# zju-pi/diff-sampler

Measured on NVIDIA H100. Metric: images/sec at fixed NFE, higher is better.
Workload: dtype fp16 operands, fp32 accumulate (split-precision: fp16 hi x hi + two e4m3 correction MMAs per product); 1 GPU; EDM cifar10 U-Net, heun num_steps=10 (NFE=18), batch 512/GPU; net=cifar10, solver=heun, nfe=18, batch_per_gpu=512, global_batch=512, weights=random init (reference constructors, seed 0), init_zero layers de-zeroed, parallelism=dp1, l2=per-forward activation working set (GBs) >> 50 MB L2

## Files before the change

### diff-sampler_b200/_cstructs.py

```python
import ctypes as C

P = C.c_uint64
I32 = C.c_int32
I64 = C.c_int64
F32 = C.c_float
F64 = C.c_double

DS_OP_GEMM, DS_OP_GN_STATS, DS_OP_GN_APPLY, DS_OP_SOFTMAX, DS_OP_POSEMB, DS_OP_LINEAR = 1, 2, 3, 4, 5, 6
DS_OP_PREP_INPUT, DS_OP_CHANMEAN, DS_OP_MEMSET, DS_OP_LAYERNORM, DS_OP_GEGLU, DS_OP_GN_FINALIZE, DS_OP_ATTN, DS_OP_EMBED = 7, 8, 9, 10, 11, 12, 13, 14
DS_OP_OPT_PREP, DS_OP_OPT_SOFTMAX, DS_OP_OPT_REDUCE, DS_OP_OPT_KNN = 15, 16, 17, 18
DS_OP_IMG_INPUT, DS_OP_IM2COL, DS_OP_POOL = 19, 20, 21
DS_OP_CLIP_INPUT, DS_OP_CLIP_HEAD = 22, 23
DS_OP_PRDC_KTH, DS_OP_PRDC_COUNT = 24, 25
DS_PRDC_KMAX, DS_PRDC_LIST = 63, 1024
DS_CLIP_GATHER, DS_CLIP_L2NORM, DS_CLIP_SCORE = 0, 1, 2
DS_POOL_MAX, DS_POOL_AVG, DS_POOL_MEAN = 0, 1, 2
DS_IO_X, DS_IO_D, DS_IO_SIGMA, DS_IO_LABELS, DS_IO_BOTTLENECK, DS_IO_CTX, DS_IO_COUNT = 0, 1, 2, 3, 4, 5, 6
DS_M_X0, DS_M_EPS, DS_M_DIV, DS_M_NONE = 0, 1, 2, 3
DS_F8_SH_A16, DS_F8_SH_LO8, DS_F8_SH_HI8 = 6, 13, 2
DS_OPT_CAP, DS_OPT_P_SHIFT, DS_OPT_BAND_NATS, DS_OPT_TAU, DS_OPT_EPS = 1024, 15, 40, 0.01, 2.0 ** -17
DS_OPT_PLAIN, DS_OPT_RESCORED, DS_OPT_UNREFINED = 0, 1, 2
DS_KNN_MAX, DS_KNN_CAND = 64, 256

SPACE_ABS, SPACE_ARENA, SPACE_WEIGHTS, SPACE_IO = 0, 1, 2, 3


def ref(space, offset):
    return (space << 60) | int(offset)


class GemmDesc(C.Structure):
    _fields_ = [
        ('a_ptr', P), ('a_dims', I64 * 4), ('a_strides', I64 * 3), ('a_box', I32 * 4), ('a_plane_n', I32),
        ('a2_ptr', P), ('a2_c', I64), ('a2_plane_n', I32), ('nkb_aux', I32),
        ('b_ptr', P), ('b_dims', I64 * 3), ('b_strides', I64 * 2), ('b_plane_batch', I32),
        ('BN', I32), ('m_tiles', I32), ('n_tiles', I32), ('num_z', I32), ('nh', I32),
# ... 104 lines not shown


class ClipInputDesc(C.Structure):
    _fields_ = [('src', P), ('tab', P), ('out', P), ('sn', I64), ('sc', I64), ('sy', I64), ('sx', I64), ('B', I32), ('H', I32), ('W', I32),
                ('S', I32), ('ky', I32), ('kx', I32), ('mean', F32 * 3), ('std', F32 * 3)]


class ClipHeadDesc(C.Structure):
    _fields_ = [('src', P), ('src2', P), ('ids', P), ('out', P), ('src_stride', I64), ('out_stride', I64), ('B', I32), ('C', I32), ('T', I32),
                ('row', I32), ('mode', I32), ('scale', F32)]


class PrdcKthDesc(C.Structure):
    _fields_ = [('part', P), ('q', P), ('t', P), ('qn2', P), ('tn2', P), ('rad', P), ('rad2', P), ('nres', P), ('ldp', I64),
                ('B', I32), ('N', I32), ('D', I32), ('nslice', I32), ('k', I32), ('pad0', I32), ('sq', F64), ('st', F64)]


class PrdcCountDesc(C.Structure):
    _fields_ = [('part', P), ('q', P), ('t', P), ('qn2', P), ('tn2', P), ('tau', P), ('tau2', P), ('rho', P), ('rho2', P), ('cnt_t', P),
                ('cnt_own', P), ('realism', P), ('nres', P), ('ldp', I64), ('B', I32), ('N', I32), ('D', I32), ('nslice', I32),
                ('sq', F64), ('st', F64), ('med', F64)]


class MemsetDesc(C.Structure):
    _fields_ = [('ptr', P), ('bytes', I64)]


class _OpUnion(C.Union):
    _fields_ = [('gemm', GemmDesc), ('gn_stats', GnStatsDesc), ('gn_apply', GnApplyDesc), ('softmax', SoftmaxDesc),
                ('posemb', PosembDesc), ('linear', LinearDesc), ('prep_input', PrepInputDesc), ('chanmean', ChanmeanDesc),
                ('memset', MemsetDesc), ('layernorm', LayernormDesc), ('geglu', GegluDesc), ('gn_finalize', GnFinalizeDesc), ('attn', AttnDesc),
                ('embed', EmbedDesc), ('opt_prep', OptPrepDesc), ('opt_softmax', OptSoftmaxDesc), ('opt_reduce', OptReduceDesc),
                ('opt_knn', OptKnnDesc), ('img_input', ImgInputDesc), ('im2col', Im2colDesc), ('pool', PoolDesc),
                ('clip_input', ClipInputDesc), ('clip_head', ClipHeadDesc), ('prdc_kth', PrdcKthDesc), ('prdc_count', PrdcCountDesc)]


class PlanOp(C.Structure):
    _fields_ = [('type', I32), ('tag', I32), ('u', _OpUnion)]


SIZEOF_CHECKS = {
    0: PlanOp, DS_OP_GEMM: GemmDesc, DS_OP_GN_STATS: GnStatsDesc, DS_OP_GN_APPLY: GnApplyDesc, DS_OP_SOFTMAX: SoftmaxDesc,
    DS_OP_POSEMB: PosembDesc, DS_OP_LINEAR: LinearDesc, DS_OP_PREP_INPUT: PrepInputDesc, DS_OP_CHANMEAN: ChanmeanDesc,
    DS_OP_MEMSET: MemsetDesc, DS_OP_LAYERNORM: LayernormDesc, DS_OP_GEGLU: GegluDesc, DS_OP_GN_FINALIZE: GnFinalizeDesc, DS_OP_ATTN: AttnDesc,
    DS_OP_EMBED: EmbedDesc, DS_OP_OPT_PREP: OptPrepDesc, DS_OP_OPT_SOFTMAX: OptSoftmaxDesc, DS_OP_OPT_REDUCE: OptReduceDesc,
    DS_OP_OPT_KNN: OptKnnDesc, DS_OP_IMG_INPUT: ImgInputDesc, DS_OP_IM2COL: Im2colDesc, DS_OP_POOL: PoolDesc,
    DS_OP_CLIP_INPUT: ClipInputDesc, DS_OP_CLIP_HEAD: ClipHeadDesc, DS_OP_PRDC_KTH: PrdcKthDesc, DS_OP_PRDC_COUNT: PrdcCountDesc,
}

UNION_FIELD = {
    DS_OP_GEMM: 'gemm', DS_OP_GN_STATS: 'gn_stats', DS_OP_GN_APPLY: 'gn_apply', DS_OP_SOFTMAX: 'softmax', DS_OP_POSEMB: 'posemb',
    DS_OP_LINEAR: 'linear', DS_OP_PREP_INPUT: 'prep_input', DS_OP_CHANMEAN: 'chanmean', DS_OP_MEMSET: 'memset',
    DS_OP_LAYERNORM: 'layernorm', DS_OP_GEGLU: 'geglu', DS_OP_GN_FINALIZE: 'gn_finalize', DS_OP_ATTN: 'attn', DS_OP_EMBED: 'embed',
}
OPT_UNION_FIELD = {DS_OP_OPT_PREP: 'opt_prep', DS_OP_OPT_SOFTMAX: 'opt_softmax', DS_OP_OPT_REDUCE: 'opt_reduce', DS_OP_OPT_KNN: 'opt_knn'}
INCEPTION_UNION_FIELD = {DS_OP_IMG_INPUT: 'img_input', DS_OP_IM2COL: 'im2col', DS_OP_POOL: 'pool'}
OPENCLIP_UNION_FIELD = {DS_OP_CLIP_INPUT: 'clip_input', DS_OP_CLIP_HEAD: 'clip_head'}
PRDC_UNION_FIELD = {DS_OP_PRDC_KTH: 'prdc_kth', DS_OP_PRDC_COUNT: 'prdc_count'}
ALL_UNION_FIELD = {**UNION_FIELD, **OPT_UNION_FIELD, **INCEPTION_UNION_FIELD, **OPENCLIP_UNION_FIELD, **PRDC_UNION_FIELD}
OP_TYPE_OF = {GemmDesc: DS_OP_GEMM, GnStatsDesc: DS_OP_GN_STATS, GnApplyDesc: DS_OP_GN_APPLY, SoftmaxDesc: DS_OP_SOFTMAX,
              PosembDesc: DS_OP_POSEMB, LinearDesc: DS_OP_LINEAR, PrepInputDesc: DS_OP_PREP_INPUT, ChanmeanDesc: DS_OP_CHANMEAN,
              MemsetDesc: DS_OP_MEMSET, LayernormDesc: DS_OP_LAYERNORM, GegluDesc: DS_OP_GEGLU, GnFinalizeDesc: DS_OP_GN_FINALIZE, AttnDesc: DS_OP_ATTN,
              EmbedDesc: DS_OP_EMBED, OptPrepDesc: DS_OP_OPT_PREP, OptSoftmaxDesc: DS_OP_OPT_SOFTMAX, OptReduceDesc: DS_OP_OPT_REDUCE,
              OptKnnDesc: DS_OP_OPT_KNN, ImgInputDesc: DS_OP_IMG_INPUT, Im2colDesc: DS_OP_IM2COL, PoolDesc: DS_OP_POOL,
              ClipInputDesc: DS_OP_CLIP_INPUT, ClipHeadDesc: DS_OP_CLIP_HEAD, PrdcKthDesc: DS_OP_PRDC_KTH, PrdcCountDesc: DS_OP_PRDC_COUNT}
```

### diff-sampler_b200/csrc/elementwise.cu

```cuda
#include "ops.h"
#include "operand.cuh"
#include <cuda_fp16.h>
#include <math.h>

namespace dsb {

__device__ __forceinline__ float silu_f(float v) { return __fdividef(v, 1.0f + __expf(-v)); }

__global__ void gn_stats_kernel(ds_gn_stats_desc d, int pix_per_cta) {
    __shared__ double s_sum[64];
    __shared__ double s_sq[64];
    const int tid = threadIdx.y * blockDim.x + threadIdx.x;
    if (tid < 64) { s_sum[tid] = 0.0; s_sq[tid] = 0.0; }
    __syncthreads();
    const int C = d.C0 + d.C1;
    const int cpg = C / d.groups;
    const int n = blockIdx.y;
    const int ncol4 = C / 4;
    const int p_begin = blockIdx.x * pix_per_cta;
    int p_end = p_begin + pix_per_cta;
    if (p_end > d.HW) p_end = d.HW;
    for (int col = threadIdx.x; col < ncol4; col += blockDim.x) {
        const int c = col * 4;
        const float* base;
// ... 513 lines not shown
    }
}

__global__ void prep_input_kernel(ds_prep_input_desc d) {
    const long long idx = (long long)blockIdx.x * blockDim.x + threadIdx.x;
    const long long total = (long long)d.B * d.HW * 8;
    if (idx >= total) return;
    const int c8 = (int)(idx & 7);
    const long long px = idx >> 3;
    const int n = (int)(px / d.HW);
    const int hw = (int)(px - (long long)n * d.HW);
    const int xb = d.x_batch > 0 ? d.x_batch : d.B;
    const int nx = n % xb;
    const float cin = d.coef[nx * d.coef_stride + 2];
    float v[8];
#pragma unroll
    for (int j = 0; j < 8; ++j) {
        const int c = c8 * 8 + j;
        v[j] = c < d.C ? cin * d.x[((long long)nx * d.C + c) * d.HW + hw] : 0.f;
    }
    store_planes<8>(reinterpret_cast<__half*>(d.out), (long long)d.B * d.HW * 64, px * 64 + c8 * 8, v, d.nplanes);
}

constexpr int VQ_CHUNK = 1024;

template <int CP>
__global__ void __launch_bounds__(256) vq_prep_input_kernel(ds_prep_input_desc d) {
    __shared__ float4 s_code[VQ_CHUNK * (CP / 4)];
    const long long px = (long long)blockIdx.x * blockDim.x + threadIdx.x;
    const long long total = (long long)d.B * d.HW;
    const bool live = px < total;
    const int n = live ? (int)(px / d.HW) : 0;
    const int hw = live ? (int)(px - (long long)n * d.HW) : 0;
    const int xb = d.x_batch > 0 ? d.x_batch : d.B;
    const int nx = n % xb;
    float v[CP];
    if (live) {
        const float cin = d.coef[nx * d.coef_stride + 2];
#pragma unroll
        for (int c = 0; c < CP; ++c) v[c] = c < d.C ? cin * d.x[((long long)nx * d.C + c) * d.HW + hw] : 0.f;
    }
    float best = INFINITY;
    int bi = 0;
    float* sc = reinterpret_cast<float*>(s_code);
    for (int base = 0; base < d.n_embed; base += VQ_CHUNK) {
        const int cnt = min(VQ_CHUNK, d.n_embed - base);
// ... 352 lines not shown
    else linear_kernel<2048><<<dim3(bx, by), wpb * 32, 0, stream>>>(*d);
    return ok();
}

OpCheck dsb::prep_input_check(const ds_prep_input_desc& d) {
    if (d.C > 64) return {-2, "prep_input: C"};
    if (d.codebook && (d.C > 8 || d.n_embed < 1)) return {-2, "prep_input: codebook"};
    return {0, nullptr};
}

extern "C" int ds_prep_input_launch(const ds_prep_input_desc* d, cudaStream_t stream) {
    if (const int rc = prep_input_check(*d).rc) return rc;
    if (d->codebook) {
        const unsigned blocks = (unsigned)(((long long)d->B * d->HW + 255) / 256);
        if (d->C <= 4) vq_prep_input_kernel<4><<<blocks, 256, 0, stream>>>(*d);
        else vq_prep_input_kernel<8><<<blocks, 256, 0, stream>>>(*d);
        return ok();
    }
    const long long total = (long long)d->B * d->HW * 8;
    prep_input_kernel<<<(unsigned)((total + 255) / 256), 256, 0, stream>>>(*d);
    return ok();
}

extern "C" int ds_chanmean_launch(const ds_chanmean_desc* d, cudaStream_t stream) {
    const int wpb = 8;
    chanmean_kernel<<<(unsigned)((d->rows + wpb - 1) / wpb), wpb * 32, 0, stream>>>(*d);
    return ok();
}
```

### diff-sampler_b200/csrc/engine.cu

```cuda
#include "../../include/diffsampler_b200.h"
#include "ops.h"
#include "ptx.cuh"
#include <cuda_fp16.h>
#include <nvtx3/nvToolsExt.h>
#include <stdio.h>
#include <stdlib.h>
#include <string.h>
#include <string>
#include <vector>

namespace dsb {
struct GemmKernelParams;
int gemm_build(const ds_gemm_desc* d, GemmKernelParams* kp);
int gemm_run(const GemmKernelParams* kp, cudaStream_t stream);
size_t gemm_params_size();
void gemm_patch_edm(GemmKernelParams* kp, const float* x, float* D);
struct AttnKernelParams;
int attn_build(const ds_attn_desc* d, AttnKernelParams* kp);
int attn_run(const AttnKernelParams* kp, cudaStream_t stream);
size_t attn_params_size();
}

static thread_local std::string g_err;

// ... 15 lines not shown
    int op;
    size_t field_off;
    int slot;
};

struct ds_unet {
    const ds_weights* w = nullptr;
    void* arena = nullptr;
    size_t arena_bytes = 0;
    std::vector<ds_plan_op> ops;
    std::vector<std::vector<unsigned char>> gemm_params;
    std::vector<IoFix> fixes;
    int last_launches = 0;
    bool profiling = false;
    std::vector<cudaEvent_t> ev0, ev1;
    std::vector<char> ev_used;
    bool graph_on = false;
    void* stage[DS_IO_COUNT] = {nullptr, nullptr, nullptr, nullptr, nullptr, nullptr};
    size_t stage_bytes[DS_IO_COUNT] = {0, 0, 0, 0, 0, 0};
    cudaGraphExec_t gexec[2] = {nullptr, nullptr};
    int gnodes[2] = {0, 0};
    int warm_runs = 0;
    cudaStream_t cap_stream = nullptr;
};

template <class F>
static void visit_ptrs(ds_plan_op& op, F f) {
#define P(field) f((void**)(void*)(&(field)))
    switch (op.type) {
        case DS_OP_GEMM: {
            ds_gemm_desc& g = op.u.gemm;
            P(g.a_ptr); P(g.a2_ptr); P(g.b_ptr); P(g.out_f32); P(g.out_h16); P(g.bias_n); P(g.bias_m); P(g.rowvec);
            P(g.residual); P(g.edm_x); P(g.edm_coef); P(g.edm_D); P(g.st_quads);
            break;
        }
        case DS_OP_GN_STATS: { auto& d = op.u.gn_stats; P(d.src0); P(d.src1); P(d.sums); break; }
        case DS_OP_GN_APPLY: {
            auto& d = op.u.gn_apply;
            P(d.src0); P(d.src1); P(d.sums); P(d.gamma); P(d.beta); P(d.ada); P(d.out_act); P(d.out_raw); P(d.out_raw_f32); P(d.coef);
            break;
        }
        case DS_OP_SOFTMAX: { auto& d = op.u.softmax; P(d.S); P(d.P); break; }
        case DS_OP_POSEMB: { auto& d = op.u.posemb; P(d.sigma); P(d.coef); P(d.emb); break; }
        case DS_OP_LINEAR: { auto& d = op.u.linear; P(d.in); P(d.W); P(d.b); P(d.add); P(d.out); break; }
        case DS_OP_PREP_INPUT: { auto& d = op.u.prep_input; P(d.x); P(d.coef); P(d.out); P(d.codebook); P(d.idx); break; }
        case DS_OP_CHANMEAN: { auto& d = op.u.chanmean; P(d.src); P(d.out); break; }
        case DS_OP_MEMSET: { auto& d = op.u.memset; P(d.ptr); break; }
        case DS_OP_LAYERNORM: { auto& d = op.u.layernorm; P(d.src); P(d.gamma); P(d.beta); P(d.out); break; }
        case DS_OP_GEGLU: { auto& d = op.u.geglu; P(d.src); P(d.out); break; }
        case DS_OP_GN_FINALIZE: { auto& d = op.u.gn_finalize; P(d.quads0); P(d.quads1); P(d.sums); P(d.gamma); P(d.beta); P(d.ada); P(d.coef); break; }
        case DS_OP_ATTN: { auto& d = op.u.attn; P(d.q); P(d.k); P(d.vt); P(d.out); break; }
        case DS_OP_EMBED: { auto& d = op.u.embed; P(d.ids); P(d.tok); P(d.pos); P(d.out); break; }
        case DS_OP_OPT_PREP: { auto& d = op.u.opt_prep; P(d.x); P(d.planes); P(d.xn2); break; }
        case DS_OP_OPT_SOFTMAX: { auto& d = op.u.opt_softmax; P(d.part); P(d.hy2); P(d.xn2); P(d.sigma); P(d.x); P(d.y); P(d.P); P(d.status); break; }
        case DS_OP_OPT_REDUCE: { auto& d = op.u.opt_reduce; P(d.part); P(d.out); break; }
        case DS_OP_OPT_KNN: { auto& d = op.u.opt_knn; P(d.part); P(d.hy2); P(d.xn2); P(d.x); P(d.y); P(d.dist); P(d.idx); break; }
        case DS_OP_IMG_INPUT: { auto& d = op.u.img_input; P(d.src); P(d.out); break; }
        case DS_OP_IM2COL: { auto& d = op.u.im2col; P(d.src); P(d.out); break; }
        case DS_OP_POOL: { auto& d = op.u.pool; P(d.src); P(d.out_f32); P(d.out_h16); break; }
        case DS_OP_CLIP_INPUT: { auto& d = op.u.clip_input; P(d.src); P(d.tab); P(d.out); break; }
        case DS_OP_CLIP_HEAD: { auto& d = op.u.clip_head; P(d.src); P(d.src2); P(d.ids); P(d.out); break; }
        case DS_OP_PRDC_KTH: {
            auto& d = op.u.prdc_kth;
            P(d.part); P(d.q); P(d.t); P(d.qn2); P(d.tn2); P(d.rad); P(d.rad2); P(d.nres);
            break;
        }
        case DS_OP_PRDC_COUNT: {
            auto& d = op.u.prdc_count;
            P(d.part); P(d.q); P(d.t); P(d.qn2); P(d.tn2); P(d.tau); P(d.tau2); P(d.rho); P(d.rho2); P(d.cnt_t); P(d.cnt_own);
            P(d.realism); P(d.nres);
            break;
        }
        default: break;
    }
#undef P
}

static dsb::OpCheck check_op(const ds_plan_op& op) {
    switch (op.type) {
        case DS_OP_GEMM: return dsb::gemm_check(op.u.gemm);
        case DS_OP_GN_STATS: return dsb::gn_stats_check(op.u.gn_stats);
        case DS_OP_GN_APPLY: return dsb::gn_apply_check(op.u.gn_apply);
        case DS_OP_LINEAR: return dsb::linear_check(op.u.linear);
        case DS_OP_PREP_INPUT: return dsb::prep_input_check(op.u.prep_input);
        case DS_OP_LAYERNORM: return dsb::layernorm_check(op.u.layernorm);
        case DS_OP_GEGLU: return dsb::geglu_check(op.u.geglu);
        case DS_OP_GN_FINALIZE: return dsb::gn_finalize_check(op.u.gn_finalize);
        case DS_OP_ATTN: return dsb::attn_check(op.u.attn);
        case DS_OP_EMBED: return dsb::embed_check(op.u.embed);
        case DS_OP_OPT_PREP: return dsb::opt_prep_check(op.u.opt_prep);
        case DS_OP_OPT_SOFTMAX: return dsb::opt_softmax_check(op.u.opt_softmax);
        case DS_OP_OPT_REDUCE: return dsb::opt_reduce_check(op.u.opt_reduce);
        case DS_OP_OPT_KNN: return dsb::opt_knn_check(op.u.opt_knn);
        case DS_OP_IMG_INPUT: return dsb::img_input_check(op.u.img_input);
        case DS_OP_IM2COL: return dsb::im2col_check(op.u.im2col);
        case DS_OP_POOL: return dsb::pool_check(op.u.pool);
        case DS_OP_CLIP_INPUT: return dsb::clip_input_check(op.u.clip_input);
        case DS_OP_CLIP_HEAD: return dsb::clip_head_check(op.u.clip_head);
        case DS_OP_PRDC_KTH: return dsb::prdc_kth_check(op.u.prdc_kth);
        case DS_OP_PRDC_COUNT: return dsb::prdc_count_check(op.u.prdc_count);
        case DS_OP_SOFTMAX: case DS_OP_POSEMB: case DS_OP_CHANMEAN: case DS_OP_MEMSET: return {0, nullptr};
        default: return {-100, "unknown op type"};
    }
}

static int launch_op(const ds_plan_op& op, const unsigned char* gemm_kp, cudaStream_t s) {
    switch (op.type) {
        case DS_OP_GEMM:
            if (gemm_kp) return dsb::gemm_run(reinterpret_cast<const dsb::GemmKernelParams*>(gemm_kp), s);
            return ds_gemm_launch(&op.u.gemm, s);
        case DS_OP_GN_STATS: return ds_gn_stats_launch(&op.u.gn_stats, s);
        case DS_OP_GN_APPLY: return ds_gn_apply_launch(&op.u.gn_apply, s);
        case DS_OP_SOFTMAX: return ds_softmax_launch(&op.u.softmax, s);
        case DS_OP_POSEMB: return ds_posemb_launch(&op.u.posemb, s);
        case DS_OP_LINEAR: return ds_linear_launch(&op.u.linear, s);
        case DS_OP_PREP_INPUT: return ds_prep_input_launch(&op.u.prep_input, s);
        case DS_OP_CHANMEAN: return ds_chanmean_launch(&op.u.chanmean, s);
        case DS_OP_LAYERNORM: return ds_layernorm_launch(&op.u.layernorm, s);
        case DS_OP_GEGLU: return ds_geglu_launch(&op.u.geglu, s);
        case DS_OP_GN_FINALIZE: return ds_gn_finalize_launch(&op.u.gn_finalize, s);
        case DS_OP_EMBED: return ds_embed_launch(&op.u.embed, s);
        case DS_OP_OPT_PREP: return ds_opt_prep_launch(&op.u.opt_prep, s);
        case DS_OP_OPT_SOFTMAX: return ds_opt_softmax_launch(&op.u.opt_softmax, s);
        case DS_OP_OPT_REDUCE: return ds_opt_reduce_launch(&op.u.opt_reduce, s);
        case DS_OP_OPT_KNN: return ds_opt_knn_launch(&op.u.opt_knn, s);
        case DS_OP_IMG_INPUT: return ds_img_input_launch(&op.u.img_input, s);
        case DS_OP_IM2COL: return ds_im2col_launch(&op.u.im2col, s);
        case DS_OP_POOL: return ds_pool_launch(&op.u.pool, s);
        case DS_OP_CLIP_INPUT: return ds_clip_input_launch(&op.u.clip_input, s);
        case DS_OP_CLIP_HEAD: return ds_clip_head_launch(&op.u.clip_head, s);
        case DS_OP_PRDC_KTH: return ds_prdc_kth_launch(&op.u.prdc_kth, s);
        case DS_OP_PRDC_COUNT: return ds_prdc_count_launch(&op.u.prdc_count, s);
        case DS_OP_ATTN:
            if (gemm_kp) return dsb::attn_run(reinterpret_cast<const dsb::AttnKernelParams*>(gemm_kp), s);
            return ds_attn_launch(&op.u.attn, s);
        case DS_OP_MEMSET:
            return cudaMemsetAsync(op.u.memset.ptr, 0, (size_t)op.u.memset.bytes, s) == cudaSuccess ? 0 : -1;
        default: return -100;
    }
}

extern "C" {

const char* ds_version(void) { return "diffsampler_b200 0.1 (sm_90a, wgmma/TMA)"; }
const char* ds_last_error(void) { return g_err.c_str(); }

int ds_weights_create(const void* host_blob, size_t bytes, ds_weights** out) {
    if (!host_blob || !out) return fail(-1, "ds_weights_create: null argument");
    ds_weights* w = new ds_weights();
    if (cudaMalloc(&w->dev, bytes ? bytes : 16) != cudaSuccess) {
        delete w;
        return fail(-2, std::string("ds_weights_create: cudaMalloc failed: ") + cudaGetErrorString(cudaGetLastError()));
    }
    if (cudaMemcpy(w->dev, host_blob, bytes, cudaMemcpyHostToDevice) != cudaSuccess) {
        cudaFree(w->dev);
        delete w;
        return fail(-3, "ds_weights_create: cudaMemcpy failed");
    }
    w->bytes = bytes;
    *out = w;
    return 0;
}

void ds_weights_destroy(ds_weights* w) {
// ... 8 lines not shown
        char buf[128];
        snprintf(buf, sizeof buf, "ds_unet_create: ds_plan_op size mismatch (caller %zu, library %zu)", op_size, sizeof(ds_plan_op));
        return fail(-4, buf);
    }
    for (int i = 0; i < n_ops; ++i) {
        const ds_plan_op& op = reinterpret_cast<const ds_plan_op*>(plan_ops)[i];
        const dsb::OpCheck c = check_op(op);
        if (c.rc) {
            char buf[160];
            snprintf(buf, sizeof buf, "ds_unet_create: op %d (type %d tag %d) refused (rc %d): %s", i, op.type, op.tag, c.rc, c.rule);
            return fail(-6, buf);
        }
    }
    ds_unet* u = new ds_unet();
    u->w = w;
    u->arena_bytes = arena_bytes;
    if (cudaMalloc(&u->arena, arena_bytes ? arena_bytes : 16) != cudaSuccess) {
        delete u;
        return fail(-2, std::string("ds_unet_create: cudaMalloc(arena) failed: ") + cudaGetErrorString(cudaGetLastError()));
    }
    cudaMemset(u->arena, 0, arena_bytes);
    u->ops.assign(reinterpret_cast<const ds_plan_op*>(plan_ops), reinterpret_cast<const ds_plan_op*>(plan_ops) + n_ops);
    u->gemm_params.resize(n_ops);
    int bad = 0;
    for (int i = 0; i < n_ops; ++i) {
        ds_plan_op& op = u->ops[i];
        visit_ptrs(op, [&](void** field) {
            const uint64_t ref = reinterpret_cast<uint64_t>(*field);
            const uint64_t space = ref >> 60;
            const uint64_t off = ref & ((1ull << 60) - 1);
            if (space == 0) return;
            if (space == 1) {
                if (off >= arena_bytes) bad = i + 1;
                *field = static_cast<char*>(u->arena) + off;
            } else if (space == 2) {
                if (off >= w->bytes) bad = i + 1;
                *field = static_cast<char*>(w->dev) + off;
            } else if (space == 3) {
                IoFix fx;
                fx.op = i;
                fx.field_off = reinterpret_cast<char*>(field) - reinterpret_cast<char*>(&op);
                fx.slot = (int)off;
                u->fixes.push_back(fx);
                *field = nullptr;
            } else {
                bad = i + 1;
            }
        });
    }
    if (bad) {
        char buf[96];
        snprintf(buf, sizeof buf, "ds_unet_create: bad pointer reference in op %d", bad - 1);
        ds_unet_destroy(u);
        return fail(-5, buf);
    }
    for (int i = 0; i < n_ops; ++i) {
        const int type = u->ops[i].type;
        if (type != DS_OP_GEMM && type != DS_OP_ATTN) continue;
        u->gemm_params[i].resize((type == DS_OP_GEMM ? dsb::gemm_params_size() : dsb::attn_params_size()) + 64);
        unsigned char* p = u->gemm_params[i].data();
        unsigned char* al = reinterpret_cast<unsigned char*>((reinterpret_cast<uintptr_t>(p) + 63) & ~uintptr_t(63));
        int rc = type == DS_OP_GEMM ? dsb::gemm_build(&u->ops[i].u.gemm, reinterpret_cast<dsb::GemmKernelParams*>(al))
                                    : dsb::attn_build(&u->ops[i].u.attn, reinterpret_cast<dsb::AttnKernelParams*>(al));
        if (rc) {
            char buf[96];
            snprintf(buf, sizeof buf, "ds_unet_create: %s failed (rc %d) for op %d tag %d", type == DS_OP_GEMM ? "gemm_build" : "attn_build", rc, i,
                     u->ops[i].tag);
            ds_unet_destroy(u);
            return fail(-6, buf);
        }
    }
    *out = u;
    return 0;
}

void ds_unet_destroy(ds_unet* u) {
    if (!u) return;
    for (auto e : u->ev0) cudaEventDestroy(e);
    for (auto e : u->ev1) cudaEventDestroy(e);
    for (int v = 0; v < 2; ++v) if (u->gexec[v]) cudaGraphExecDestroy(u->gexec[v]);
    for (int k = 0; k < DS_IO_COUNT; ++k) if (u->stage[k]) cudaFree(u->stage[k]);
    if (u->cap_stream) cudaStreamDestroy(u->cap_stream);
    cudaFree(u->arena);
    delete u;
}

int ds_unet_forward_io(ds_unet* u, const void* const* io_in, int n_io, void* stream);

int ds_unet_forward(ds_unet* u, const float* x, const float* sigma, const float* labels, float* out_D, float* out_bottleneck,
                    void* stream) {
    const void* io[DS_IO_COUNT] = {x, out_D, sigma, labels, out_bottleneck, nullptr};
    return ds_unet_forward_io(u, io, DS_IO_COUNT, stream);
}

static int run_ops(ds_unet* u, const void* const* io, cudaStream_t s, bool profiling) {
    for (const IoFix& fx : u->fixes) {
        if (fx.slot < 0 || fx.slot >= DS_IO_COUNT) return fail(-7, "ds_unet_forward: bad io slot");
        void** field = reinterpret_cast<void**>(reinterpret_cast<char*>(&u->ops[fx.op]) + fx.field_off);
        *field = const_cast<void*>(io[fx.slot]);
    }
    int launches = 0;
    for (size_t i = 0; i < u->ops.size(); ++i) {
        ds_plan_op& op = u->ops[i];
        const unsigned char* kp = nullptr;
        if (op.type == DS_OP_GEMM || op.type == DS_OP_ATTN) {
            unsigned char* p = u->gemm_params[i].data();
            unsigned char* al = reinterpret_cast<unsigned char*>((reinterpret_cast<uintptr_t>(p) + 63) & ~uintptr_t(63));
            if (op.type == DS_OP_GEMM && op.u.gemm.edm_out)
                dsb::gemm_patch_edm(reinterpret_cast<dsb::GemmKernelParams*>(al), op.u.gemm.edm_x, op.u.gemm.edm_D);
            kp = al;
        }
        if (op.type == DS_OP_CHANMEAN && op.u.chanmean.out == nullptr) continue;
        if (profiling) { cudaEventRecord(u->ev0[i], s); u->ev_used[i] = 1; }
        int rc = launch_op(op, kp, s);
        if (profiling) cudaEventRecord(u->ev1[i], s);
        if (rc) {
            char buf[160];
            snprintf(buf, sizeof buf, "ds_unet_forward: op %zu (type %d tag %d) failed rc=%d cuda=%s", i, op.type, op.tag, rc,
                     cudaGetErrorString(cudaGetLastError()));
            return fail(-8, buf);
        }
        ++launches;
    }
    return launches;
}

static int build_graph(ds_unet* u, int variant, const void* const* staged_io) {
    if (!u->cap_stream && cudaStreamCreateWithFlags(&u->cap_stream, cudaStreamNonBlocking) != cudaSuccess)
        return fail(-20, "ds_unet_forward: cannot create the capture stream");
    if (cudaStreamBeginCapture(u->cap_stream, cudaStreamCaptureModeThreadLocal) != cudaSuccess)
        return fail(-21, std::string("ds_unet_forward: cudaStreamBeginCapture failed: ") + cudaGetErrorString(cudaGetLastError()));
    const int n = run_ops(u, staged_io, u->cap_stream, false);
    cudaGraph_t g = nullptr;
    const cudaError_t e = cudaStreamEndCapture(u->cap_stream, &g);
    if (n < 0 || e != cudaSuccess || !g) {
        if (g) cudaGraphDestroy(g);
        if (n < 0) return n;
        return fail(-22, std::string("ds_unet_forward: stream capture failed: ") + cudaGetErrorString(e));
    }
    cudaGraphExec_t ex = nullptr;
    const cudaError_t ei = cudaGraphInstantiate(&ex, g, 0);
    cudaGraphDestroy(g);
    if (ei != cudaSuccess) return fail(-23, std::string("ds_unet_forward: cudaGraphInstantiate failed: ") + cudaGetErrorString(ei));
    u->gexec[variant] = ex;
    u->gnodes[variant] = n;
// ... 146 lines not shown
        case DS_OP_GN_APPLY: return sizeof(ds_gn_apply_desc);
        case DS_OP_SOFTMAX: return sizeof(ds_softmax_desc);
        case DS_OP_POSEMB: return sizeof(ds_posemb_desc);
        case DS_OP_LINEAR: return sizeof(ds_linear_desc);
        case DS_OP_PREP_INPUT: return sizeof(ds_prep_input_desc);
        case DS_OP_CHANMEAN: return sizeof(ds_chanmean_desc);
        case DS_OP_MEMSET: return sizeof(ds_memset_desc);
        case DS_OP_LAYERNORM: return sizeof(ds_layernorm_desc);
        case DS_OP_GEGLU: return sizeof(ds_geglu_desc);
        case DS_OP_GN_FINALIZE: return sizeof(ds_gn_finalize_desc);
        case DS_OP_ATTN: return sizeof(ds_attn_desc);
        case DS_OP_EMBED: return sizeof(ds_embed_desc);
        case DS_OP_OPT_PREP: return sizeof(ds_opt_prep_desc);
        case DS_OP_OPT_SOFTMAX: return sizeof(ds_opt_softmax_desc);
        case DS_OP_OPT_REDUCE: return sizeof(ds_opt_reduce_desc);
        case DS_OP_OPT_KNN: return sizeof(ds_opt_knn_desc);
        case DS_OP_IMG_INPUT: return sizeof(ds_img_input_desc);
        case DS_OP_IM2COL: return sizeof(ds_im2col_desc);
        case DS_OP_POOL: return sizeof(ds_pool_desc);
        case DS_OP_CLIP_INPUT: return sizeof(ds_clip_input_desc);
        case DS_OP_CLIP_HEAD: return sizeof(ds_clip_head_desc);
        case DS_OP_PRDC_KTH: return sizeof(ds_prdc_kth_desc);
        case DS_OP_PRDC_COUNT: return sizeof(ds_prdc_count_desc);
        default: return 0;
    }
}

int ds_gits_cost(const float* traj, const float* eps, const float* t_steps, double* out, int N, int B, int64_t n_per_sample, void* stream) {
    ds_gits_cost_desc d;
    d.traj = traj; d.eps = eps; d.t = t_steps; d.out = out; d.N = N; d.B = B; d.n = n_per_sample;
    int rc = ds_gits_cost_launch(&d, static_cast<cudaStream_t>(stream));
    if (rc) return fail(rc, std::string("ds_gits_cost: launch failed: ") + cudaGetErrorString(cudaGetLastError()));
    return 0;
}

int ds_amed_predict(const float* weights, const int* dims6, const float* bottleneck, const float* t_cur, const float* t_next,
                    float scale_dir, float scale_time, float* out4, int B, void* stream) {
    if (!weights || !dims6 || !t_cur || !t_next || !out4) return fail(-1, "ds_amed_predict: null argument");
    NvtxRange nvtx_range("ds_amed_predict");
    int rc = ds_amed_predict_launch(weights, dims6, bottleneck, t_cur, t_next, scale_dir, scale_time, out4, B, static_cast<cudaStream_t>(stream));
    if (rc) return fail(rc, std::string("ds_amed_predict: launch failed: ") + cudaGetErrorString(cudaGetLastError()));
    return 0;
}

int ds_images_to_uint8(const float* images, unsigned char* out, int B, int C, int HW, void* stream) {
    if (!images || !out) return fail(-1, "ds_images_to_uint8: null argument");
// ... 32 lines not shown
```

### diff-sampler_b200/csrc/ops.h

```cpp
#pragma once
#include <stdint.h>
#include <cuda_runtime.h>

#ifdef __cplusplus
extern "C" {
#endif

enum { DS_F8_SH_A16 = 6, DS_F8_SH_LO8 = 13, DS_F8_SH_HI8 = 2 };
typedef struct ds_gemm_desc {
    const void* a_ptr;
    int64_t a_dims[4];
    int64_t a_strides[3];
    int32_t a_box[4];
    int32_t a_plane_n;
    const void* a2_ptr;
    int64_t a2_c;
    int32_t a2_plane_n;
    int32_t nkb_aux;
    const void* b_ptr;
    int64_t b_dims[3];
    int64_t b_strides[2];
    int32_t b_plane_batch;
    int32_t BN;
    int32_t m_tiles, n_tiles, num_z, nh;
// ... 137 lines not shown
    const float* add;
    int64_t add_stride;
    float* out;
    int32_t n_rows, in_f, out_f;
    int32_t act;
    float in_scale;
    int32_t pad0;
} ds_linear_desc;

typedef struct ds_prep_input_desc {
    const float* x;
    const float* coef;
    int32_t coef_stride;
    int32_t B, C, HW;
    int32_t nplanes;
    int32_t x_batch;
    void* out;
    const float* codebook;
    int32_t* idx;
    int32_t n_embed;
    int32_t pad0;
} ds_prep_input_desc;

typedef struct ds_layernorm_desc {
    const float* src;
    const float* gamma;
    const float* beta;
    void* out;
    int64_t rows;
    int32_t C;
    int32_t nplanes;
    float eps;
    int32_t fmt;
} ds_layernorm_desc;

typedef struct ds_geglu_desc {
    const float* src;
    void* out;
    int64_t rows;
    int32_t I;
    int32_t nplanes;
    int32_t fmt;
    int32_t mode;
} ds_geglu_desc;

typedef struct ds_embed_desc {
// ... 205 lines not shown
int ds_clip_head_launch(const ds_clip_head_desc* d, cudaStream_t stream);
int ds_img_input_launch(const ds_img_input_desc* d, cudaStream_t stream);
int ds_im2col_launch(const ds_im2col_desc* d, cudaStream_t stream);
int ds_pool_launch(const ds_pool_desc* d, cudaStream_t stream);

int ds_opt_prep_launch(const ds_opt_prep_desc* d, cudaStream_t stream);
int ds_opt_softmax_launch(const ds_opt_softmax_desc* d, cudaStream_t stream);
int ds_opt_reduce_launch(const ds_opt_reduce_desc* d, cudaStream_t stream);
int ds_opt_knn_launch(const ds_opt_knn_desc* d, cudaStream_t stream);
int ds_amed_predict_launch(const float* w, const int* dims6, const float* bott, const float* t_cur, const float* t_next, float scale_dir,
                           float scale_time, float* out, int B, cudaStream_t stream);
int ds_to_uint8_launch(const float* x, unsigned char* out, int B, int Cc, int HW, cudaStream_t stream);
int ds_update_launch(const ds_update_desc* d, cudaStream_t stream);
int ds_threshold_launch(const ds_threshold_desc* d, cudaStream_t stream);
int ds_gn_stats_launch(const ds_gn_stats_desc* d, cudaStream_t stream);
int ds_gn_apply_launch(const ds_gn_apply_desc* d, cudaStream_t stream);
int ds_gn_finalize_launch(const ds_gn_finalize_desc* d, cudaStream_t stream);
int ds_attn_launch(const ds_attn_desc* d, cudaStream_t stream);
int ds_softmax_launch(const ds_softmax_desc* d, cudaStream_t stream);
int ds_posemb_launch(const ds_posemb_desc* d, cudaStream_t stream);
int ds_linear_launch(const ds_linear_desc* d, cudaStream_t stream);
int ds_prep_input_launch(const ds_prep_input_desc* d, cudaStream_t stream);
int ds_chanmean_launch(const ds_chanmean_desc* d, cudaStream_t stream);
int ds_layernorm_launch(const ds_layernorm_desc* d, cudaStream_t stream);
int ds_geglu_launch(const ds_geglu_desc* d, cudaStream_t stream);
int ds_embed_launch(const ds_embed_desc* d, cudaStream_t stream);

enum { DS_OP_GEMM = 1, DS_OP_GN_STATS = 2, DS_OP_GN_APPLY = 3, DS_OP_SOFTMAX = 4, DS_OP_POSEMB = 5, DS_OP_LINEAR = 6,
       DS_OP_PREP_INPUT = 7, DS_OP_CHANMEAN = 8, DS_OP_MEMSET = 9, DS_OP_LAYERNORM = 10, DS_OP_GEGLU = 11,
       DS_OP_GN_FINALIZE = 12, DS_OP_ATTN = 13, DS_OP_EMBED = 14, DS_OP_OPT_PREP = 15, DS_OP_OPT_SOFTMAX = 16,
       DS_OP_OPT_REDUCE = 17, DS_OP_OPT_KNN = 18, DS_OP_IMG_INPUT = 19, DS_OP_IM2COL = 20, DS_OP_POOL = 21,
       DS_OP_CLIP_INPUT = 22, DS_OP_CLIP_HEAD = 23, DS_OP_PRDC_KTH = 24, DS_OP_PRDC_COUNT = 25 };
enum { DS_IO_X = 0, DS_IO_D = 1, DS_IO_SIGMA = 2, DS_IO_LABELS = 3, DS_IO_BOTTLENECK = 4, DS_IO_CTX = 5, DS_IO_COUNT = 6 };

typedef struct ds_memset_desc {
    void* ptr;
    int64_t bytes;
} ds_memset_desc;

typedef struct ds_plan_op {
    int32_t type;
    int32_t tag;
    union {
        ds_gemm_desc gemm;
        ds_gn_stats_desc gn_stats;
        ds_gn_apply_desc gn_apply;
        ds_softmax_desc softmax;
        ds_posemb_desc posemb;
        ds_linear_desc linear;
        ds_prep_input_desc prep_input;
        ds_chanmean_desc chanmean;
        ds_memset_desc memset;
        ds_layernorm_desc layernorm;
        ds_geglu_desc geglu;
        ds_gn_finalize_desc gn_finalize;
        ds_attn_desc attn;
        ds_embed_desc embed;
        ds_opt_prep_desc opt_prep;
        ds_opt_softmax_desc opt_softmax;
        ds_opt_reduce_desc opt_reduce;
        ds_opt_knn_desc opt_knn;
        ds_img_input_desc img_input;
        ds_im2col_desc im2col;
        ds_pool_desc pool;
        ds_clip_input_desc clip_input;
        ds_clip_head_desc clip_head;
        ds_prdc_kth_desc prdc_kth;
        ds_prdc_count_desc prdc_count;
    } u;
} ds_plan_op;

#ifdef __cplusplus
}

namespace dsb {
struct OpCheck {
    int rc;
    const char* rule;
};
OpCheck gemm_check(const ds_gemm_desc& d);
OpCheck attn_check(const ds_attn_desc& d);
OpCheck gn_stats_check(const ds_gn_stats_desc& d);
OpCheck gn_finalize_check(const ds_gn_finalize_desc& d);
OpCheck gn_apply_check(const ds_gn_apply_desc& d);
OpCheck embed_check(const ds_embed_desc& d);
OpCheck layernorm_check(const ds_layernorm_desc& d);
OpCheck geglu_check(const ds_geglu_desc& d);
OpCheck linear_check(const ds_linear_desc& d);
OpCheck prep_input_check(const ds_prep_input_desc& d);
OpCheck opt_prep_check(const ds_opt_prep_desc& d);
OpCheck opt_softmax_check(const ds_opt_softmax_desc& d);
OpCheck opt_reduce_check(const ds_opt_reduce_desc& d);
OpCheck opt_knn_check(const ds_opt_knn_desc& d);
OpCheck img_input_check(const ds_img_input_desc& d);
OpCheck im2col_check(const ds_im2col_desc& d);
OpCheck pool_check(const ds_pool_desc& d);
OpCheck clip_input_check(const ds_clip_input_desc& d);
OpCheck clip_head_check(const ds_clip_head_desc& d);
OpCheck prdc_kth_check(const ds_prdc_kth_desc& d);
OpCheck prdc_count_check(const ds_prdc_count_desc& d);
}
#endif
```

Measured before the change: 297.1 images/s.

## Split final 3x3 output conv into single-tap GEMM plus tap-gather epilogue

The final output conv (3x3, few output channels) with EDM epilogue is detected at build time. Its weights are repacked so one taps=1 GEMM produces all 9*C per-tap partial products per pixel into an fp32 scratch buffer. A new gather kernel then sums the shifted neighbours, adds the bias and applies the EDM skip/out coefficients. This avoids the 9-tap implicit-GEMM loop over a tiny N tile, but adds an extra kernel launch and an fp32 scratch write and read.

```diff
diff --git a/diff-sampler_b200/_cstructs.py b/diff-sampler_b200/_cstructs.py
--- a/diff-sampler_b200/_cstructs.py
+++ b/diff-sampler_b200/_cstructs.py
@@ -12,6 +12,8 @@
 DS_OP_IMG_INPUT, DS_OP_IM2COL, DS_OP_POOL = 19, 20, 21
 DS_OP_CLIP_INPUT, DS_OP_CLIP_HEAD = 22, 23
 DS_OP_PRDC_KTH, DS_OP_PRDC_COUNT = 24, 25
+DS_OP_TAP_GATHER = 26
+DS_TAP_GATHER_CMAX = 8
 DS_PRDC_KMAX, DS_PRDC_LIST = 63, 1024
 DS_CLIP_GATHER, DS_CLIP_L2NORM, DS_CLIP_SCORE = 0, 1, 2
 DS_POOL_MAX, DS_POOL_AVG, DS_POOL_MEAN = 0, 1, 2
@@ -162,6 +164,11 @@
                 ('sq', F64), ('st', F64), ('med', F64)]
 
 
+class TapGatherDesc(C.Structure):
+    _fields_ = [('P', P), ('bias', P), ('x', P), ('coef', P), ('D', P), ('ldp', I64), ('B', I32), ('H', I32), ('W', I32), ('C', I32),
+                ('coef_stride', I32), ('pad0', I32)]
+
+
 class MemsetDesc(C.Structure):
     _fields_ = [('ptr', P), ('bytes', I64)]
 
@@ -172,7 +179,8 @@
                 ('memset', MemsetDesc), ('layernorm', LayernormDesc), ('geglu', GegluDesc), ('gn_finalize', GnFinalizeDesc), ('attn', AttnDesc),
                 ('embed', EmbedDesc), ('opt_prep', OptPrepDesc), ('opt_softmax', OptSoftmaxDesc), ('opt_reduce', OptReduceDesc),
                 ('opt_knn', OptKnnDesc), ('img_input', ImgInputDesc), ('im2col', Im2colDesc), ('pool', PoolDesc),
-                ('clip_input', ClipInputDesc), ('clip_head', ClipHeadDesc), ('prdc_kth', PrdcKthDesc), ('prdc_count', PrdcCountDesc)]
+                ('clip_input', ClipInputDesc), ('clip_head', ClipHeadDesc), ('prdc_kth', PrdcKthDesc), ('prdc_count', PrdcCountDesc),
+                ('tap_gather', TapGatherDesc)]
 
 
 class PlanOp(C.Structure):
@@ -186,6 +194,7 @@
     DS_OP_EMBED: EmbedDesc, DS_OP_OPT_PREP: OptPrepDesc, DS_OP_OPT_SOFTMAX: OptSoftmaxDesc, DS_OP_OPT_REDUCE: OptReduceDesc,
     DS_OP_OPT_KNN: OptKnnDesc, DS_OP_IMG_INPUT: ImgInputDesc, DS_OP_IM2COL: Im2colDesc, DS_OP_POOL: PoolDesc,
     DS_OP_CLIP_INPUT: ClipInputDesc, DS_OP_CLIP_HEAD: ClipHeadDesc, DS_OP_PRDC_KTH: PrdcKthDesc, DS_OP_PRDC_COUNT: PrdcCountDesc,
+    DS_OP_TAP_GATHER: TapGatherDesc,
 }
 
 UNION_FIELD = {
@@ -197,10 +206,12 @@
 INCEPTION_UNION_FIELD = {DS_OP_IMG_INPUT: 'img_input', DS_OP_IM2COL: 'im2col', DS_OP_POOL: 'pool'}
 OPENCLIP_UNION_FIELD = {DS_OP_CLIP_INPUT: 'clip_input', DS_OP_CLIP_HEAD: 'clip_head'}
 PRDC_UNION_FIELD = {DS_OP_PRDC_KTH: 'prdc_kth', DS_OP_PRDC_COUNT: 'prdc_count'}
-ALL_UNION_FIELD = {**UNION_FIELD, **OPT_UNION_FIELD, **INCEPTION_UNION_FIELD, **OPENCLIP_UNION_FIELD, **PRDC_UNION_FIELD}
+EXEC_UNION_FIELD = {DS_OP_TAP_GATHER: 'tap_gather'}
+ALL_UNION_FIELD = {**UNION_FIELD, **OPT_UNION_FIELD, **INCEPTION_UNION_FIELD, **OPENCLIP_UNION_FIELD, **PRDC_UNION_FIELD, **EXEC_UNION_FIELD}
 OP_TYPE_OF = {GemmDesc: DS_OP_GEMM, GnStatsDesc: DS_OP_GN_STATS, GnApplyDesc: DS_OP_GN_APPLY, SoftmaxDesc: DS_OP_SOFTMAX,
               PosembDesc: DS_OP_POSEMB, LinearDesc: DS_OP_LINEAR, PrepInputDesc: DS_OP_PREP_INPUT, ChanmeanDesc: DS_OP_CHANMEAN,
               MemsetDesc: DS_OP_MEMSET, LayernormDesc: DS_OP_LAYERNORM, GegluDesc: DS_OP_GEGLU, GnFinalizeDesc: DS_OP_GN_FINALIZE, AttnDesc: DS_OP_ATTN,
               EmbedDesc: DS_OP_EMBED, OptPrepDesc: DS_OP_OPT_PREP, OptSoftmaxDesc: DS_OP_OPT_SOFTMAX, OptReduceDesc: DS_OP_OPT_REDUCE,
               OptKnnDesc: DS_OP_OPT_KNN, ImgInputDesc: DS_OP_IMG_INPUT, Im2colDesc: DS_OP_IM2COL, PoolDesc: DS_OP_POOL,
-              ClipInputDesc: DS_OP_CLIP_INPUT, ClipHeadDesc: DS_OP_CLIP_HEAD, PrdcKthDesc: DS_OP_PRDC_KTH, PrdcCountDesc: DS_OP_PRDC_COUNT}
+              ClipInputDesc: DS_OP_CLIP_INPUT, ClipHeadDesc: DS_OP_CLIP_HEAD, PrdcKthDesc: DS_OP_PRDC_KTH, PrdcCountDesc: DS_OP_PRDC_COUNT,
+              TapGatherDesc: DS_OP_TAP_GATHER}
diff --git a/diff-sampler_b200/csrc/elementwise.cu b/diff-sampler_b200/csrc/elementwise.cu
--- a/diff-sampler_b200/csrc/elementwise.cu
+++ b/diff-sampler_b200/csrc/elementwise.cu
@@ -559,6 +559,35 @@
     store_planes<8>(reinterpret_cast<__half*>(d.out), (long long)d.B * d.HW * 64, px * 64 + c8 * 8, v, d.nplanes);
 }
 
+__global__ void __launch_bounds__(256) tap_gather_kernel(ds_tap_gather_desc d) {
+    const long long px = (long long)blockIdx.x * blockDim.x + threadIdx.x;
+    const int HW = d.H * d.W;
+    if (px >= (long long)d.B * HW) return;
+    const int n = (int)(px / HW);
+    const int hw = (int)(px - (long long)n * HW);
+    const int h = hw / d.W, w = hw - h * d.W;
+    float acc[DS_TAP_GATHER_CMAX];
+#pragma unroll
+    for (int c = 0; c < DS_TAP_GATHER_CMAX; ++c) acc[c] = 0.f;
+#pragma unroll
+    for (int t = 0; t < 9; ++t) {
+        const int hh = h + t / 3 - 1, ww = w + t % 3 - 1;
+        if (hh < 0 || hh >= d.H || ww < 0 || ww >= d.W) continue;
+        const float* p = d.P + (px + (long long)(t / 3 - 1) * d.W + (t % 3 - 1)) * d.ldp + t * d.C;
+#pragma unroll
+        for (int c = 0; c < DS_TAP_GATHER_CMAX; ++c)
+            if (c < d.C) acc[c] += __ldg(p + c);
+    }
+    const float cskip = __ldg(d.coef + n * d.coef_stride + 0);
+    const float cout = __ldg(d.coef + n * d.coef_stride + 1);
+#pragma unroll
+    for (int c = 0; c < DS_TAP_GATHER_CMAX; ++c) {
+        if (c >= d.C) break;
+        const long long idx = ((long long)n * d.C + c) * HW + hw;
+        d.D[idx] = cskip * __ldg(d.x + idx) + cout * (acc[c] + __ldg(d.bias + c));
+    }
+}
+
 constexpr int VQ_CHUNK = 1024;
 
 template <int CP>
@@ -957,6 +986,21 @@
     return ok();
 }
 
+OpCheck dsb::tap_gather_check(const ds_tap_gather_desc& d) {
+    if (!d.P || !d.bias || !d.x || !d.coef || !d.D) return {-2, "tap_gather: pointers"};
+    if (d.B < 1 || d.H < 1 || d.W < 1) return {-2, "tap_gather: shape"};
+    if (d.C < 1 || d.C > DS_TAP_GATHER_CMAX || d.ldp < 9 * d.C) return {-2, "tap_gather: C"};
+    if (d.coef_stride != 0 && d.coef_stride != 4) return {-2, "tap_gather: coef_stride"};
+    return {0, nullptr};
+}
+
+extern "C" int ds_tap_gather_launch(const ds_tap_gather_desc* d, cudaStream_t stream) {
+    if (const int rc = tap_gather_check(*d).rc) return rc;
+    const long long total = (long long)d->B * d->H * d->W;
+    tap_gather_kernel<<<(unsigned)((total + 255) / 256), 256, 0, stream>>>(*d);
+    return ok();
+}
+
 extern "C" int ds_chanmean_launch(const ds_chanmean_desc* d, cudaStream_t stream) {
     const int wpb = 8;
     chanmean_kernel<<<(unsigned)((d->rows + wpb - 1) / wpb), wpb * 32, 0, stream>>>(*d);
diff --git a/diff-sampler_b200/csrc/engine.cu b/diff-sampler_b200/csrc/engine.cu
--- a/diff-sampler_b200/csrc/engine.cu
+++ b/diff-sampler_b200/csrc/engine.cu
@@ -61,6 +61,9 @@
     int gnodes[2] = {0, 0};
     int warm_runs = 0;
     cudaStream_t cap_stream = nullptr;
+    std::vector<float*> head_p;
+    std::vector<int> head_ldp;
+    std::vector<void*> owned;
 };
 
 template <class F>
@@ -84,6 +87,7 @@
         case DS_OP_LINEAR: { auto& d = op.u.linear; P(d.in); P(d.W); P(d.b); P(d.add); P(d.out); break; }
         case DS_OP_PREP_INPUT: { auto& d = op.u.prep_input; P(d.x); P(d.coef); P(d.out); P(d.codebook); P(d.idx); break; }
         case DS_OP_CHANMEAN: { auto& d = op.u.chanmean; P(d.src); P(d.out); break; }
+        case DS_OP_TAP_GATHER: { auto& d = op.u.tap_gather; P(d.P); P(d.bias); P(d.x); P(d.coef); P(d.D); break; }
         case DS_OP_MEMSET: { auto& d = op.u.memset; P(d.ptr); break; }
         case DS_OP_LAYERNORM: { auto& d = op.u.layernorm; P(d.src); P(d.gamma); P(d.beta); P(d.out); break; }
         case DS_OP_GEGLU: { auto& d = op.u.geglu; P(d.src); P(d.out); break; }
@@ -122,6 +126,7 @@
         case DS_OP_GN_APPLY: return dsb::gn_apply_check(op.u.gn_apply);
         case DS_OP_LINEAR: return dsb::linear_check(op.u.linear);
         case DS_OP_PREP_INPUT: return dsb::prep_input_check(op.u.prep_input);
+        case DS_OP_TAP_GATHER: return dsb::tap_gather_check(op.u.tap_gather);
         case DS_OP_LAYERNORM: return dsb::layernorm_check(op.u.layernorm);
         case DS_OP_GEGLU: return dsb::geglu_check(op.u.geglu);
         case DS_OP_GN_FINALIZE: return dsb::gn_finalize_check(op.u.gn_finalize);
@@ -155,6 +160,7 @@
         case DS_OP_LINEAR: return ds_linear_launch(&op.u.linear, s);
         case DS_OP_PREP_INPUT: return ds_prep_input_launch(&op.u.prep_input, s);
         case DS_OP_CHANMEAN: return ds_chanmean_launch(&op.u.chanmean, s);
+        case DS_OP_TAP_GATHER: return ds_tap_gather_launch(&op.u.tap_gather, s);
         case DS_OP_LAYERNORM: return ds_layernorm_launch(&op.u.layernorm, s);
         case DS_OP_GEGLU: return ds_geglu_launch(&op.u.geglu, s);
         case DS_OP_GN_FINALIZE: return ds_gn_finalize_launch(&op.u.gn_finalize, s);
@@ -179,6 +185,77 @@
     }
 }
 
+static int head_rows(const ds_gemm_desc& g) {
+    if (g.a_mode != 0 || g.taps != 9 || g.edm_out != 1 || g.num_z != 1 || g.a2_c != 0 || g.n_tiles != 1) return 0;
+    if (g.edm_C < 1 || g.edm_C > DS_TAP_GATHER_CMAX || g.n_valid != g.edm_C || !g.bias_n || !g.edm_coef) return 0;
+    if (g.residual || g.rowvec || g.bias_m || g.st_quads || g.relu || g.scale != 1.f || g.conv_H < 1 || g.conv_W < 1) return 0;
+    if (g.m_valid % (g.conv_H * g.conv_W) != 0) return 0;
+    for (int t = 0; t < 9; ++t)
+        if (g.tap_dh[t] != t / 3 - 1 || g.tap_dw[t] != t % 3 - 1 || g.tap_cb[t] != 0) return 0;
+    const int n = 9 * g.edm_C;
+    return n <= 32 ? 32 : (n <= 64 ? 64 : 0);
+}
+
+static bool repack_plane(char* dst, const char* src, int64_t w, int C, int esz) {
+    for (int t = 0; t < 9; ++t)
+        if (cudaMemcpy2D(dst + (int64_t)t * C * w * esz, w * esz, src + (int64_t)t * w * esz, 9 * w * esz, w * esz, C,
+                         cudaMemcpyDeviceToDevice) != cudaSuccess)
+            return false;
+    return true;
+}
+
+static int split_head(ds_unet* u, int i, unsigned char* kp) {
+    const ds_gemm_desc& g = u->ops[i].u.gemm;
+    const int rows = head_rows(g);
+    const int C = g.edm_C, f8 = g.f8 & 1;
+    const int64_t cpad = (int64_t)g.cpb * 64, c128 = (int64_t)((g.cpb + 1) / 2) * 128, cout_pad = g.b_dims[1];
+    const int np16 = f8 ? 1 : (int)g.b_dims[2];
+    const size_t wbytes = (size_t)np16 * rows * cpad * 2 + (f8 ? (size_t)2 * rows * c128 : 0);
+    void* wbuf = nullptr;
+    float* part = nullptr;
+    if (cudaMalloc(&wbuf, wbytes) != cudaSuccess) return -2;
+    u->owned.push_back(wbuf);
+    if (cudaMalloc(&part, (size_t)g.m_valid * rows * sizeof(float)) != cudaSuccess) return -2;
+    u->owned.push_back(part);
+    if (cudaMemset(wbuf, 0, wbytes) != cudaSuccess) return -3;
+    const char* src = static_cast<const char*>(g.b_ptr);
+    char* dst = static_cast<char*>(wbuf);
+    for (int p = 0; p < np16; ++p)
+        if (!repack_plane(dst + (int64_t)p * rows * cpad * 2, src + (int64_t)p * cout_pad * 9 * cpad * 2, cpad, C, 2)) return -3;
+    if (f8) {
+        const char* s8 = src + cout_pad * 9 * cpad * 2;
+        char* d8 = dst + (int64_t)rows * cpad * 2;
+        for (int p = 0; p < 2; ++p)
+            if (!repack_plane(d8 + (int64_t)p * rows * c128, s8 + (int64_t)p * cout_pad * 9 * c128, c128, C, 1)) return -3;
+    }
+    if (cudaDeviceSynchronize() != cudaSuccess) return -3;
+    ds_gemm_desc g1 = g;
+    g1.taps = 1;
+    memset(g1.tap_dh, 0, sizeof g1.tap_dh);
+    memset(g1.tap_dw, 0, sizeof g1.tap_dw);
+    memset(g1.tap_cb, 0, sizeof g1.tap_cb);
+    g1.b_ptr = wbuf;
+    g1.b_dims[0] = cpad; g1.b_dims[1] = rows; g1.b_dims[2] = np16;
+    g1.b_strides[0] = cpad * 2; g1.b_strides[1] = rows * cpad * 2;
+    g1.BN = rows; g1.n_tiles = 1; g1.n_valid = 9 * C;
+    g1.out_f32 = part; g1.out_h16 = nullptr; g1.o_plane = 0; g1.ldo = rows;
+    g1.bias_n = nullptr;
+    g1.edm_out = 0; g1.edm_x = nullptr; g1.edm_coef = nullptr; g1.edm_D = nullptr;
+    if (const int rc = dsb::gemm_build(&g1, reinterpret_cast<dsb::GemmKernelParams*>(kp))) return rc;
+    u->head_p[i] = part;
+    u->head_ldp[i] = rows;
+    return 0;
+}
+
+static int run_split_head(const ds_gemm_desc& g, const unsigned char* kp, float* part, int ldp, cudaStream_t s) {
+    if (const int rc = dsb::gemm_run(reinterpret_cast<const dsb::GemmKernelParams*>(kp), s)) return rc;
+    ds_tap_gather_desc t;
+    memset(&t, 0, sizeof t);
+    t.P = part; t.bias = g.bias_n; t.x = g.edm_x; t.coef = g.edm_coef; t.D = g.edm_D; t.ldp = ldp;
+    t.B = g.m_valid / (g.conv_H * g.conv_W); t.H = g.conv_H; t.W = g.conv_W; t.C = g.edm_C; t.coef_stride = g.edm_coef_stride;
+    return ds_tap_gather_launch(&t, s);
+}
+
 extern "C" {
 
 const char* ds_version(void) { return "diffsampler_b200 0.1 (sm_90a, wgmma/TMA)"; }
@@ -233,6 +310,8 @@
     cudaMemset(u->arena, 0, arena_bytes);
     u->ops.assign(reinterpret_cast<const ds_plan_op*>(plan_ops), reinterpret_cast<const ds_plan_op*>(plan_ops) + n_ops);
     u->gemm_params.resize(n_ops);
+    u->head_p.assign(n_ops, nullptr);
+    u->head_ldp.assign(n_ops, 0);
     int bad = 0;
     for (int i = 0; i < n_ops; ++i) {
         ds_plan_op& op = u->ops[i];
@@ -271,7 +350,8 @@
         u->gemm_params[i].resize((type == DS_OP_GEMM ? dsb::gemm_params_size() : dsb::attn_params_size()) + 64);
         unsigned char* p = u->gemm_params[i].data();
         unsigned char* al = reinterpret_cast<unsigned char*>((reinterpret_cast<uintptr_t>(p) + 63) & ~uintptr_t(63));
-        int rc = type == DS_OP_GEMM ? dsb::gemm_build(&u->ops[i].u.gemm, reinterpret_cast<dsb::GemmKernelParams*>(al))
+        int rc = type == DS_OP_GEMM ? (head_rows(u->ops[i].u.gemm) ? split_head(u, i, al)
+                                                                   : dsb::gemm_build(&u->ops[i].u.gemm, reinterpret_cast<dsb::GemmKernelParams*>(al)))
                                     : dsb::attn_build(&u->ops[i].u.attn, reinterpret_cast<dsb::AttnKernelParams*>(al));
         if (rc) {
             char buf[96];
@@ -292,6 +372,7 @@
     for (int v = 0; v < 2; ++v) if (u->gexec[v]) cudaGraphExecDestroy(u->gexec[v]);
     for (int k = 0; k < DS_IO_COUNT; ++k) if (u->stage[k]) cudaFree(u->stage[k]);
     if (u->cap_stream) cudaStreamDestroy(u->cap_stream);
+    for (void* p : u->owned) cudaFree(p);
     cudaFree(u->arena);
     delete u;
 }
@@ -317,13 +398,14 @@
         if (op.type == DS_OP_GEMM || op.type == DS_OP_ATTN) {
             unsigned char* p = u->gemm_params[i].data();
             unsigned char* al = reinterpret_cast<unsigned char*>((reinterpret_cast<uintptr_t>(p) + 63) & ~uintptr_t(63));
-            if (op.type == DS_OP_GEMM && op.u.gemm.edm_out)
+            if (op.type == DS_OP_GEMM && op.u.gemm.edm_out && !u->head_p[i])
                 dsb::gemm_patch_edm(reinterpret_cast<dsb::GemmKernelParams*>(al), op.u.gemm.edm_x, op.u.gemm.edm_D);
             kp = al;
         }
         if (op.type == DS_OP_CHANMEAN && op.u.chanmean.out == nullptr) continue;
         if (profiling) { cudaEventRecord(u->ev0[i], s); u->ev_used[i] = 1; }
-        int rc = launch_op(op, kp, s);
+        const bool split = u->head_p[i] != nullptr;
+        int rc = split ? run_split_head(op.u.gemm, kp, u->head_p[i], u->head_ldp[i], s) : launch_op(op, kp, s);
         if (profiling) cudaEventRecord(u->ev1[i], s);
         if (rc) {
             char buf[160];
@@ -331,7 +413,7 @@
                      cudaGetErrorString(cudaGetLastError()));
             return fail(-8, buf);
         }
-        ++launches;
+        launches += split ? 2 : 1;
     }
     return launches;
 }
@@ -524,6 +606,7 @@
         case DS_OP_CLIP_HEAD: return sizeof(ds_clip_head_desc);
         case DS_OP_PRDC_KTH: return sizeof(ds_prdc_kth_desc);
         case DS_OP_PRDC_COUNT: return sizeof(ds_prdc_count_desc);
+        case DS_OP_TAP_GATHER: return sizeof(ds_tap_gather_desc);
         default: return 0;
     }
 }
diff --git a/diff-sampler_b200/csrc/ops.h b/diff-sampler_b200/csrc/ops.h
--- a/diff-sampler_b200/csrc/ops.h
+++ b/diff-sampler_b200/csrc/ops.h
@@ -183,6 +183,19 @@
     int32_t pad0;
 } ds_prep_input_desc;
 
+enum { DS_TAP_GATHER_CMAX = 8 };
+typedef struct ds_tap_gather_desc {
+    const float* P;
+    const float* bias;
+    const float* x;
+    const float* coef;
+    float* D;
+    int64_t ldp;
+    int32_t B, H, W, C;
+    int32_t coef_stride;
+    int32_t pad0;
+} ds_tap_gather_desc;
+
 typedef struct ds_layernorm_desc {
     const float* src;
     const float* gamma;
@@ -434,6 +447,7 @@
 int ds_linear_launch(const ds_linear_desc* d, cudaStream_t stream);
 int ds_prep_input_launch(const ds_prep_input_desc* d, cudaStream_t stream);
 int ds_chanmean_launch(const ds_chanmean_desc* d, cudaStream_t stream);
+int ds_tap_gather_launch(const ds_tap_gather_desc* d, cudaStream_t stream);
 int ds_layernorm_launch(const ds_layernorm_desc* d, cudaStream_t stream);
 int ds_geglu_launch(const ds_geglu_desc* d, cudaStream_t stream);
 int ds_embed_launch(const ds_embed_desc* d, cudaStream_t stream);
@@ -442,7 +456,8 @@
        DS_OP_PREP_INPUT = 7, DS_OP_CHANMEAN = 8, DS_OP_MEMSET = 9, DS_OP_LAYERNORM = 10, DS_OP_GEGLU = 11,
        DS_OP_GN_FINALIZE = 12, DS_OP_ATTN = 13, DS_OP_EMBED = 14, DS_OP_OPT_PREP = 15, DS_OP_OPT_SOFTMAX = 16,
        DS_OP_OPT_REDUCE = 17, DS_OP_OPT_KNN = 18, DS_OP_IMG_INPUT = 19, DS_OP_IM2COL = 20, DS_OP_POOL = 21,
-       DS_OP_CLIP_INPUT = 22, DS_OP_CLIP_HEAD = 23, DS_OP_PRDC_KTH = 24, DS_OP_PRDC_COUNT = 25 };
+       DS_OP_CLIP_INPUT = 22, DS_OP_CLIP_HEAD = 23, DS_OP_PRDC_KTH = 24, DS_OP_PRDC_COUNT = 25,
+       DS_OP_TAP_GATHER = 26 };
 enum { DS_IO_X = 0, DS_IO_D = 1, DS_IO_SIGMA = 2, DS_IO_LABELS = 3, DS_IO_BOTTLENECK = 4, DS_IO_CTX = 5, DS_IO_COUNT = 6 };
 
 typedef struct ds_memset_desc {
@@ -479,6 +494,7 @@
         ds_clip_head_desc clip_head;
         ds_prdc_kth_desc prdc_kth;
         ds_prdc_count_desc prdc_count;
+        ds_tap_gather_desc tap_gather;
     } u;
 } ds_plan_op;
 
@@ -500,6 +516,7 @@
 OpCheck geglu_check(const ds_geglu_desc& d);
 OpCheck linear_check(const ds_linear_desc& d);
 OpCheck prep_input_check(const ds_prep_input_desc& d);
+OpCheck tap_gather_check(const ds_tap_gather_desc& d);
 OpCheck opt_prep_check(const ds_opt_prep_desc& d);
 OpCheck opt_softmax_check(const ds_opt_softmax_desc& d);
 OpCheck opt_reduce_check(const ds_opt_reduce_desc& d);
```

New measurement: 298.3 images/s (median of 6 runs). Within noise of the previous version (+0.4%).
